# jkulhanek/wild-gaussians

Hardware: AMD Instinct MI355X
Metric: train_iters_per_s (fwd+bwd of the rasterizer, 1M Gaussians @1080p) (higher is better)
Workload: dtype f32

## Files before the change

wild-gaussians_amd/csrc/wg_sort.h:

```cpp
#pragma once
#include "wg_common.h"

namespace wg {

__device__ __forceinline__ void bitonic_ce(uint64_t* skeys, uint32_t t, uint32_t j, uint32_t k) {
    const uint32_t i = ((t & ~(j - 1)) << 1) | (t & (j - 1));
    const uint32_t l = i | j;
    const uint64_t a = skeys[i], b = skeys[l];
    const bool ascending = (i & k) == 0;
    if ((a > b) == ascending) {
        skeys[i] = b;
        skeys[l] = a;
    }
}

template <int D>
__device__ __forceinline__ uint32_t lane_xor(uint32_t v) {
    if constexpr (D == 1) return (uint32_t)__builtin_amdgcn_update_dpp(0, (int)v, 0xB1, 0xF, 0xF, false);
    else if constexpr (D == 2) return (uint32_t)__builtin_amdgcn_update_dpp(0, (int)v, 0x4E, 0xF, 0xF, false);
    else if constexpr (D == 8) return (uint32_t)__builtin_amdgcn_update_dpp(0, (int)v, 0x128, 0xF, 0xF, false);
    else if constexpr (D == 4) return (uint32_t)__builtin_amdgcn_ds_swizzle((int)v, 0x101F);
    else if constexpr (D == 16) return (uint32_t)__builtin_amdgcn_ds_swizzle((int)v, 0x401F);
    else return (uint32_t)__shfl_xor((int)v, 32);
}

template <int E>
struct SortCtx {
    uint64_t key[E];
    uint32_t t;
    uint32_t gidx;
    uint64_t* xchg;
};

__device__ __forceinline__ void keep(uint64_t& mine, uint64_t other, bool keep_min) {
    const bool other_less = other < mine;
    mine = (other_less == keep_min) ? other : mine;
}

template <int E, int K, int J>
__device__ __forceinline__ void sort_stage(SortCtx<E>& c) {
    if constexpr (J < E) {
#pragma unroll
        for (int r = 0; r < E; r++) {
            if ((r & J) == 0) {
                const bool asc = ((c.gidx + r) & K) == 0;
                uint64_t& a = c.key[r];
                uint64_t& b = c.key[r | J];
                if ((a > b) == asc) {
                    const uint64_t tmp = a;
                    a = b;
                    b = tmp;
                }
            }
        }
    } else {
        const bool asc = (c.gidx & K) == 0;
        const bool lower = (c.t & (J / E)) == 0;
        const bool keep_min = lower == asc;
        if constexpr (J < 64 * E) {
#pragma unroll
            for (int r = 0; r < E; r++) {
                const uint32_t lo = lane_xor<J / E>((uint32_t)c.key[r]);
                const uint32_t hi = lane_xor<J / E>((uint32_t)(c.key[r] >> 32));
                keep(c.key[r], ((uint64_t)hi << 32) | lo, keep_min);
            }
        } else {
#ifndef WG_SORT_XCHG_TRANSPOSED
#define WG_SORT_XCHG_TRANSPOSED 1
#endif
            constexpr uint32_t RS = WG_SORT_XCHG_TRANSPOSED ? 256u : 1u, TS = WG_SORT_XCHG_TRANSPOSED ? 1u : (uint32_t)E;
            uint64_t* mine = c.xchg + TS * c.t;
#pragma unroll
            for (int r = 0; r < E; r++) mine[RS * r] = c.key[r];
            __syncthreads();
            const uint64_t* theirs = c.xchg + TS * (c.t ^ (J / E));
            uint64_t other[E];
#pragma unroll
            for (int r = 0; r < E; r++) other[r] = theirs[RS * r];
            __syncthreads();
#pragma unroll
            for (int r = 0; r < E; r++) keep(c.key[r], other[r], keep_min);
        }
    }
}

template <int E, int K, int J>
__device__ __forceinline__ void sort_stages(SortCtx<E>& c) {
    sort_stage<E, K, J>(c);
    if constexpr (J > 1) sort_stages<E, K, J / 2>(c);
}

template <int E, int K>
__device__ __forceinline__ void sort_levels(SortCtx<E>& c, uint32_t kmax) {
    if constexpr (K > 2) sort_levels<E, K / 2>(c, kmax);
    if (K <= kmax) sort_stages<E, K, K / 2>(c);
}

template <int E>
__device__ __forceinline__ void tile_sort_body(uint64_t* skeys, uint32_t n, const uint32_t* src, const float* __restrict__ depths,
                                               uint32_t* dst, uint32_t id_mask) {
    uint32_t np2 = E;
    while (np2 < n) np2 <<= 1;
    SortCtx<E> c;
    c.t = threadIdx.x;
    c.gidx = E * threadIdx.x;
    c.xchg = skeys;
#pragma unroll
    for (int r = 0; r < E; r++) {
        const uint32_t i = c.gidx + r;
        uint64_t key = ~0ull;
        if (i < n) {
            const uint32_t id = src[i] & id_mask;
            key = ((uint64_t)__float_as_uint(depths[id]) << 32) | id;
        }
        c.key[r] = key;
    }
    __syncthreads();
    sort_levels<E, 256 * E>(c, np2);
    __syncthreads();
#pragma unroll
    for (int r = 0; r < E; r++)
        if (c.gidx + r < n) dst[c.gidx + r] = (uint32_t)c.key[r];
}

__device__ __forceinline__ uint64_t depth_key(const float* __restrict__ depths, uint32_t id) {
    return ((uint64_t)__float_as_uint(depths[id]) << 32) | id;
}

__device__ __forceinline__ uint32_t depth_code(uint32_t depth_bits, uint32_t cb) {
    const uint32_t near_bits = 0x3E4CCCCDu;
    if (cb == 0u || depth_bits <= near_bits) return 0u;
    return min((1u << cb) - 1u, (depth_bits - near_bits) >> (27u - cb));
}
__device__ __forceinline__ uint32_t code_bits_of(uint32_t id_mask) { return 32u - (uint32_t)__builtin_popcount(id_mask); }
constexpr int MIN_ID_BITS = 20, MAX_ID_BITS_CODED = 24;

constexpr uint32_t FRONT_CAP = 2048;

struct SelectScratch {
    uint64_t sample[256];
    uint64_t sorted[256];
    uint32_t ids[FRONT_CAP];
    uint32_t count;
    uint32_t nvalid;
};

__device__ __forceinline__ uint32_t extract_pass(const uint32_t* __restrict__ bag, uint32_t n, const float* __restrict__ depths, uint64_t lo,
                                                 uint64_t thr, uint32_t cap, uint32_t id_mask, SelectScratch& sc) {
    const uint32_t tid = threadIdx.x;
    const uint32_t cb = code_bits_of(id_mask);
    const bool coded = cb != 0u;
    const uint32_t code_shift = coded ? 32u - cb : 0u;
    const int c_lo = lo == 0ull ? -1 : (int)depth_code((uint32_t)(lo >> 32), cb);
    const int c_hi = thr == ~0ull ? (1 << 16) : (int)depth_code((uint32_t)(thr >> 32), cb);
    __syncthreads();
    if (tid == 0) sc.count = 0;
    __syncthreads();
    constexpr uint32_t U = 8;
    for (uint32_t base = 0; base < n; base += 256 * U) {
        uint32_t id[U];
        uint32_t inside = 0;
        uint64_t key[U];
#pragma unroll
        for (uint32_t u = 0; u < U; u++) {
            const uint32_t i = base + u * 256 + tid;
            uint32_t e = 0u;
            bool valid = false;
            if (i < n) { e = bag[i]; valid = true; }
            id[u] = e & id_mask;
            const int c = (int)(e >> code_shift);
            const bool sure = valid && coded && c > c_lo && c < c_hi;
            const bool maybe = valid && (!coded || c == c_lo || c == c_hi);
            if (sure) inside |= 1u << u;
            key[u] = maybe ? depth_key(depths, id[u]) : 0ull;
        }
#pragma unroll
        for (uint32_t u = 0; u < U; u++) {
            if (base + u * 256 >= n) break;
            const bool in = ((inside >> u) & 1u) || (key[u] > lo && key[u] <= thr);
            const uint64_t m = __ballot(in);
            if (m != 0ull) {
                const int leader = __builtin_ctzll(m);
                uint32_t wbase = 0;
                if ((int)(tid & 63) == leader) wbase = atomicAdd(&sc.count, (uint32_t)__builtin_popcountll(m));
                wbase = (uint32_t)__builtin_amdgcn_readlane((int)wbase, leader);
                const uint32_t pos = wbase + __builtin_amdgcn_mbcnt_hi((uint32_t)(m >> 32), __builtin_amdgcn_mbcnt_lo((uint32_t)m, 0u));
                if (in && pos < cap) sc.ids[pos] = id[u];
            }
        }
    }
    __syncthreads();
    return sc.count;
}

__device__ __forceinline__ uint32_t extract_front(const uint32_t* __restrict__ bag, uint32_t n, const float* __restrict__ depths, uint64_t lo,
                                                  uint32_t remaining, uint32_t target, uint32_t cap, uint32_t id_mask, SelectScratch& sc) {
    const uint32_t tid = threadIdx.x;
    if (remaining <= cap) return extract_pass(bag, n, depths, lo, ~0ull, cap, id_mask, sc);
    const uint64_t mine = depth_key(depths, bag[(uint32_t)(((uint64_t)tid * n) >> 8)] & id_mask);
    const bool valid = mine > lo;
    __syncthreads();
    sc.sample[tid] = valid ? mine : ~0ull;
    if (tid == 0) sc.nvalid = 0;
    __syncthreads();
    if (valid) atomicAdd(&sc.nvalid, 1u);
    if (tid < 64) {
        SortCtx<4> c;
        c.t = tid;
        c.gidx = 4 * tid;
        c.xchg = nullptr;
#pragma unroll
        for (int r = 0; r < 4; r++) c.key[r] = sc.sample[4 * tid + r];
        sort_levels<4, 256>(c, 256u);
#pragma unroll
        for (int r = 0; r < 4; r++) sc.sorted[4 * tid + r] = c.key[r];
    }
    __syncthreads();
    const uint32_t k = sc.nvalid;
    for (;;) {
        uint64_t thr;
        if (k > 0 && target > 0) {
            thr = sc.sorted[min(k - 1, (uint32_t)(((uint64_t)k * target) / remaining))];
        } else {
            uint64_t best = ~0ull;
            for (uint32_t i = tid; i < n; i += 256) {
                const uint64_t key = depth_key(depths, bag[i] & id_mask);
                if (key > lo) best = min(best, key);
            }
            __syncthreads();
            sc.sample[tid] = best;
            __syncthreads();
            for (uint32_t j = 0; j < 256; j++) best = min(best, sc.sample[j]);
            thr = best;
        }
        const uint32_t F = extract_pass(bag, n, depths, lo, thr, cap, id_mask, sc);
        if (F <= cap) return F;
        target >>= 1;
    }
}

}
```

Baseline: 1086.

## Use wave-uniform ballot masks for bitonic compare-exchange direction and batch key loads

Rewrites the per-tile bitonic sort's compare-exchange so that swap and keep decisions are computed as 64-bit wave ballots XORed with compile-time or wave-uniform lane masks, then applied via inverse ballot in batches of up to four. The aim is to replace per-lane direction arithmetic and divergent selects with scalar-mask operations. It also switches DPP lane swaps to mov_dpp with bound_ctrl, and restructures the initial key gather so that all id loads are issued before the depth loads. The added complexity risks higher SGPR pressure and subtle correctness issues in the direction masks.

Result: no change. 1093 (median of 6 runs) (+0.6%).

```diff
diff --git a/wild-gaussians_amd/csrc/wg_sort.h b/wild-gaussians_amd/csrc/wg_sort.h
--- a/wild-gaussians_amd/csrc/wg_sort.h
+++ b/wild-gaussians_amd/csrc/wg_sort.h
@@ -16,9 +16,9 @@
 
 template <int D>
 __device__ __forceinline__ uint32_t lane_xor(uint32_t v) {
-    if constexpr (D == 1) return (uint32_t)__builtin_amdgcn_update_dpp(0, (int)v, 0xB1, 0xF, 0xF, false);
-    else if constexpr (D == 2) return (uint32_t)__builtin_amdgcn_update_dpp(0, (int)v, 0x4E, 0xF, 0xF, false);
-    else if constexpr (D == 8) return (uint32_t)__builtin_amdgcn_update_dpp(0, (int)v, 0x128, 0xF, 0xF, false);
+    if constexpr (D == 1) return (uint32_t)__builtin_amdgcn_mov_dpp((int)v, 0xB1, 0xF, 0xF, true);
+    else if constexpr (D == 2) return (uint32_t)__builtin_amdgcn_mov_dpp((int)v, 0x4E, 0xF, 0xF, true);
+    else if constexpr (D == 8) return (uint32_t)__builtin_amdgcn_mov_dpp((int)v, 0x128, 0xF, 0xF, true);
     else if constexpr (D == 4) return (uint32_t)__builtin_amdgcn_ds_swizzle((int)v, 0x101F);
     else if constexpr (D == 16) return (uint32_t)__builtin_amdgcn_ds_swizzle((int)v, 0x401F);
     else return (uint32_t)__shfl_xor((int)v, 32);
@@ -28,41 +28,83 @@
 struct SortCtx {
     uint64_t key[E];
     uint32_t t;
+    uint32_t wave;
     uint32_t gidx;
     uint64_t* xchg;
 };
 
-__device__ __forceinline__ void keep(uint64_t& mine, uint64_t other, bool keep_min) {
-    const bool other_less = other < mine;
-    mine = (other_less == keep_min) ? other : mine;
+template <int E>
+__device__ __forceinline__ void sort_ctx_init(SortCtx<E>& c, uint64_t* xchg) {
+    c.t = threadIdx.x;
+    c.wave = (uint32_t)__builtin_amdgcn_readfirstlane((int)(threadIdx.x >> 6));
+    c.gidx = E * threadIdx.x;
+    c.xchg = xchg;
+}
+
+constexpr uint64_t lanes_with_bit_clear(uint32_t b) {
+    uint64_t m = 0;
+    for (uint32_t l = 0; l < 64; l++)
+        if ((l & b) == 0) m |= 1ull << l;
+    return m;
+}
+
+template <uint32_t B>
+__device__ __forceinline__ uint64_t thread_bit_clear_mask(uint32_t wave) {
+    if constexpr (B < 64) return lanes_with_bit_clear(B);
+    else if constexpr (B < 256) return (wave & (B / 64)) == 0 ? ~0ull : 0ull;
+    else return ~0ull;
+}
+
+template <int B>
+__device__ __forceinline__ void keep_batch(uint64_t* mine, const uint64_t* other, uint64_t keep_max_m) {
+    uint64_t take_m[B];
+#pragma unroll
+    for (int i = 0; i < B; i++) take_m[i] = __builtin_amdgcn_ballot_w64(other[i] < mine[i]) ^ keep_max_m;
+#pragma unroll
+    for (int i = 0; i < B; i++) mine[i] = __builtin_amdgcn_inverse_ballot_w64(take_m[i]) ? other[i] : mine[i];
 }
 
 template <int E, int K, int J>
 __device__ __forceinline__ void sort_stage(SortCtx<E>& c) {
+    constexpr int B = E < 4 ? E : 4;
     if constexpr (J < E) {
-#pragma unroll
-        for (int r = 0; r < E; r++) {
-            if ((r & J) == 0) {
-                const bool asc = ((c.gidx + r) & K) == 0;
-                uint64_t& a = c.key[r];
-                uint64_t& b = c.key[r | J];
-                if ((a > b) == asc) {
-                    const uint64_t tmp = a;
-                    a = b;
-                    b = tmp;
+        int first[E / 2];
+        int pairs = 0;
+#pragma unroll
+        for (int r = 0; r < E; r++)
+            if ((r & J) == 0) first[pairs++] = r;
+#pragma unroll
+        for (int g = 0; g < E / 2; g += B) {
+            uint64_t swap_m[B];
+#pragma unroll
+            for (int i = 0; i < B && g + i < E / 2; i++) {
+                const int r = first[g + i];
+                const uint64_t a = c.key[r], b = c.key[r | J];
+                if constexpr (K < E) swap_m[i] = (r & K) == 0 ? __builtin_amdgcn_ballot_w64(a > b) : __builtin_amdgcn_ballot_w64(a <= b);
+                else swap_m[i] = __builtin_amdgcn_ballot_w64(a > b) ^ ~thread_bit_clear_mask<K / E>(c.wave);
+            }
+#pragma unroll
+            for (int i = 0; i < B && g + i < E / 2; i++) {
+                const int r = first[g + i];
+                const uint64_t a = c.key[r], b = c.key[r | J];
+                const bool swap = __builtin_amdgcn_inverse_ballot_w64(swap_m[i]);
+                c.key[r] = swap ? b : a;
+                c.key[r | J] = swap ? a : b;
+            }
+        }
+    } else {
+        const uint64_t keep_max_m = thread_bit_clear_mask<J / E>(c.wave) ^ thread_bit_clear_mask<K / E>(c.wave);
+        if constexpr (J < 64 * E) {
+#pragma unroll
+            for (int g = 0; g < E; g += B) {
+                uint64_t other[B];
+#pragma unroll
+                for (int i = 0; i < B; i++) {
+                    const uint32_t lo = lane_xor<J / E>((uint32_t)c.key[g + i]);
+                    const uint32_t hi = lane_xor<J / E>((uint32_t)(c.key[g + i] >> 32));
+                    other[i] = ((uint64_t)hi << 32) | lo;
                 }
-            }
-        }
-    } else {
-        const bool asc = (c.gidx & K) == 0;
-        const bool lower = (c.t & (J / E)) == 0;
-        const bool keep_min = lower == asc;
-        if constexpr (J < 64 * E) {
-#pragma unroll
-            for (int r = 0; r < E; r++) {
-                const uint32_t lo = lane_xor<J / E>((uint32_t)c.key[r]);
-                const uint32_t hi = lane_xor<J / E>((uint32_t)(c.key[r] >> 32));
-                keep(c.key[r], ((uint64_t)hi << 32) | lo, keep_min);
+                keep_batch<B>(&c.key[g], other, keep_max_m);
             }
         } else {
 #ifndef WG_SORT_XCHG_TRANSPOSED
@@ -79,7 +121,7 @@
             for (int r = 0; r < E; r++) other[r] = theirs[RS * r];
             __syncthreads();
 #pragma unroll
-            for (int r = 0; r < E; r++) keep(c.key[r], other[r], keep_min);
+            for (int g = 0; g < E; g += B) keep_batch<B>(&c.key[g], &other[g], keep_max_m);
         }
     }
 }
@@ -102,18 +144,21 @@
     uint32_t np2 = E;
     while (np2 < n) np2 <<= 1;
     SortCtx<E> c;
-    c.t = threadIdx.x;
-    c.gidx = E * threadIdx.x;
-    c.xchg = skeys;
-#pragma unroll
-    for (int r = 0; r < E; r++) {
-        const uint32_t i = c.gidx + r;
-        uint64_t key = ~0ull;
-        if (i < n) {
-            const uint32_t id = src[i] & id_mask;
-            key = ((uint64_t)__float_as_uint(depths[id]) << 32) | id;
-        }
-        c.key[r] = key;
+    sort_ctx_init(c, skeys);
+    if (n != 0u) {
+        uint32_t id[E], depth_bits[E];
+#pragma unroll
+        for (int r = 0; r < E; r++) id[r] = src[min(c.gidx + r, n - 1u)] & id_mask;
+#pragma unroll
+        for (int r = 0; r < E; r++) depth_bits[r] = __float_as_uint(depths[id[r]]);
+#pragma unroll
+        for (int r = 0; r < E; r++) {
+            asm volatile("" : "+v"(depth_bits[r]));
+            c.key[r] = c.gidx + r < n ? ((uint64_t)depth_bits[r] << 32) | id[r] : ~0ull;
+        }
+    } else {
+#pragma unroll
+        for (int r = 0; r < E; r++) c.key[r] = ~0ull;
     }
     __syncthreads();
     sort_levels<E, 256 * E>(c, np2);
@@ -206,9 +251,7 @@
     if (valid) atomicAdd(&sc.nvalid, 1u);
     if (tid < 64) {
         SortCtx<4> c;
-        c.t = tid;
-        c.gidx = 4 * tid;
-        c.xchg = nullptr;
+        sort_ctx_init(c, nullptr);
 #pragma unroll
         for (int r = 0; r < 4; r++) c.key[r] = sc.sample[4 * tid + r];
         sort_levels<4, 256>(c, 256u);
```
